# thiviyanT/ARK

Hardware: AMD Instinct MI355X
Metric: training graphs/sec (higher is better)
Workload: dtype f16 fwd / bf16 bwd MFMA operands (BASELINE configs[1] says bf16: bf16 forward operands miss the 1e-4 ELBO bar, fp16 has the same width and MFMA rate), f32 accumulate+state; 1 GPU; autoreg_syn-paths SAIL train step (fwd+ELBO+bwd+Adam; batches resident in HBM); batch_per_gpu=1024, global_batch=1024, d_model=512, d_latent=10, n_layers=3, seq_len=11, vocab=55, hipgraph=True, launch=hipGraph replay, settle_steps=300, parallelism=dp1

## Files before the change

### ark_amd/csrc/embed.hip

```cpp
#include "common.h"
#include "../../include/ark_amd.h"

namespace ark {

__device__ __forceinline__ void put16x4(void* base, long idx4, f32x4 v, int prec) {
  if (prec == PREC_F16) {
    typedef _Float16 h4 __attribute__((ext_vector_type(4)));
    auto c = [](float x) { return (_Float16)fminf(fmaxf(x, -65504.0f), 65504.0f); };
    reinterpret_cast<h4*>(base)[idx4] = h4{c(v[0]), c(v[1]), c(v[2]), c(v[3])};
  } else {
    typedef __bf16 b4 __attribute__((ext_vector_type(4)));
    reinterpret_cast<b4*>(base)[idx4] = b4{(__bf16)v[0], (__bf16)v[1], (__bf16)v[2], (__bf16)v[3]};
  }
}

__device__ __forceinline__ void enc_pool_fwd_body(int b, const int64_t* __restrict__ triples, const float* __restrict__ E,
                                                           const float* __restrict__ R, float* __restrict__ g,
                                                           float* __restrict__ inv_cnt, int T, int D, long pad_rid,
                                                           void* g16a, int prec_a, void* g16b, int prec_b) {
  const int64_t* tr = triples + (long)b * T * 3;
  int cnt = 0;
  for (int t = 0; t < T; ++t) cnt += (pad_rid < 0 || tr[t * 3 + 1] != pad_rid) ? 1 : 0;
  const float w = 1.0f / (float)(pad_rid < 0 ? T : (cnt > 0 ? cnt : 1));
  if (threadIdx.x == 0 && inv_cnt) inv_cnt[b] = w;
// ... 191 lines not shown
      id[k] = 0; srow[k] = 0; sc[k] = 0.f;
      ok[k] = (i + k < i1) && scatter_item(p, i + k, id[k], srow[k], sc[k]) && col_ok;
    }
#pragma unroll
    for (int k = 0; k < U; ++k) v[k] = ok[k] ? p.src[srow[k] * p.ld_src + p.col_off + c0 + lane] : 0.f;
#pragma unroll
    for (int k = 0; k < U; ++k)
      if (ok[k]) atomicAdd(&tab[id[k] * 64 + lane], sc[k] * v[k]);
  }
  __syncthreads();
  if (col_ok)
    for (int r = wave; r < p.n_rows; r += 4) {
      const float v = tab[r * 64 + lane];
      if (v != 0.f) atomicAdd(&p.dst[(long)r * p.D + c0 + lane], v);
    }
}

__global__ __launch_bounds__(256) void scatter_global_kernel(ScatterArgs p) {
  const int lane = threadIdx.x & 63;
  const int wave_global = blockIdx.x * 4 + (threadIdx.x >> 6);
  const int n_waves = gridDim.x * 4;
  for (int i = wave_global; i < p.n_items; i += n_waves) {
    long id, srow; float sc;
    if (!scatter_item(p, i, id, srow, sc)) continue;
    const float* s = p.src + srow * p.ld_src + p.col_off;
    float* d = p.dst + id * p.D;
    for (int c = lane; c < p.D; c += 64) {
      const float v = sc * s[c];
      if (v != 0.f) atomicAdd(&d[c], v);
    }
  }
}

__global__ __launch_bounds__(256) void enc_scatter_fused_kernel(const int64_t* __restrict__ triples, const float* __restrict__ dg,
                                                                const float* __restrict__ inv_cnt, float* __restrict__ dE,
                                                                float* __restrict__ dR, int B, int T, int D, int n_ent, int n_rel,
                                                                long pad_eid, long pad_rid, int n_chunks) {
  ARK_CHAIN_PRIO();
  extern __shared__ __attribute__((aligned(16))) char smem[];
  float* te = reinterpret_cast<float*>(smem);
  float* tr = te + (size_t)n_ent * 64;
  const int slice = blockIdx.x / n_chunks, chunk = blockIdx.x % n_chunks;
  const int c0 = slice * 64;
  const int lane = threadIdx.x & 63, wave = threadIdx.x >> 6;
  for (int i = threadIdx.x; i < (n_ent + n_rel) * 64; i += 256) te[i] = 0.f;
  __syncthreads();
  const int n_items = B * T;
  const int per = (n_items + n_chunks - 1) / n_chunks;
  const int i0 = chunk * per, i1 = min(n_items, i0 + per);
  const bool col_ok = (c0 + lane) < D;
  constexpr int U = 4;
  for (int i = i0 + wave * U; i < i1; i += 4 * U) {
    long h[U], r[U], t[U]; float sc[U], vh[U], vr[U], vt[U]; bool ok[U];
#pragma unroll
    for (int k = 0; k < U; ++k) {
      const int it = min(i + k, i1 - 1);
      const int64_t* p3 = triples + (long)it * 3;
      h[k] = p3[0]; r[k] = p3[1]; t[k] = p3[2];
      ok[k] = (i + k < i1) && col_ok && !(pad_rid >= 0 && r[k] == pad_rid);
      sc[k] = inv_cnt[it / T];
    }
#pragma unroll
    for (int k = 0; k < U; ++k) {
      const int it = min(i + k, i1 - 1);
      const float* src = dg + (long)(it / T) * 3 * D + c0 + lane;
      vh[k] = ok[k] ? src[0] : 0.f; vr[k] = ok[k] ? src[D] : 0.f; vt[k] = ok[k] ? src[2 * D] : 0.f;
    }
#pragma unroll
    for (int k = 0; k < U; ++k)
      if (ok[k]) {
        if (h[k] != pad_eid) atomicAdd(&te[h[k] * 64 + lane], sc[k] * vh[k]);
        if (r[k] != pad_rid) atomicAdd(&tr[r[k] * 64 + lane], sc[k] * vr[k]);
        if (t[k] != pad_eid) atomicAdd(&te[t[k] * 64 + lane], sc[k] * vt[k]);
      }
  }
  __syncthreads();
  if (col_ok) {
    for (int row = wave; row < n_ent; row += 4) {
      const float v = te[row * 64 + lane];
      if (v != 0.f) atomicAdd(&dE[(long)row * D + c0 + lane], v);
    }
    for (int row = wave; row < n_rel; row += 4) {
      const float v = tr[row * 64 + lane];
      if (v != 0.f) atomicAdd(&dR[(long)row * D + c0 + lane], v);
    }
  }
}

#ifndef ARK_SCATTER_CHUNK
#define ARK_SCATTER_CHUNK 48
#endif
constexpr int g_scatter_chunk_items = ARK_SCATTER_CHUNK;

static int launch_scatter(const ScatterArgs& p, hipStream_t st) {
  if (p.n_items <= 0) return 0;
  if ((long)p.n_rows * 64 * 4 <= 48 * 1024) {
    const int slices = (p.D + 63) / 64;
    int n_chunks = (p.n_items + g_scatter_chunk_items - 1) / g_scatter_chunk_items;
    if (n_chunks > 2048 / slices) n_chunks = 2048 / slices;
    if (n_chunks < 1) n_chunks = 1;
    hipLaunchKernelGGL(scatter_lds_kernel, dim3(slices * n_chunks), dim3(256), (size_t)p.n_rows * 64 * 4, st, p, n_chunks);
  } else {
    int grid = (p.n_items + 3) / 4; if (grid > 2048) grid = 2048;
    hipLaunchKernelGGL(scatter_global_kernel, dim3(grid), dim3(256), 0, st, p);
  }
  ARK_LAUNCH_CHECK();
  return 0;
}

}

extern "C" int ark_enc_pool_fwd(const int64_t* triples, const float* E, const float* R, float* g, float* inv_cnt,
                                int B, int T, int D, int64_t pad_rid, void* stream) {
  using namespace ark;
  if (!triples || !E || !R || !g || B <= 0 || T <= 0 || D <= 0) return ARK_ERR_ARG;
  if (D % 4 != 0) return ARK_ERR_SHAPE;
  hipLaunchKernelGGL(enc_pool_fwd_kernel, dim3(B), dim3(256), 0, (hipStream_t)stream, triples, E, R, g, inv_cnt, T, D,
// ... 28 lines not shown
  if (x16a && (g16b == nullptr) != (x16b == nullptr)) return ARK_ERR_ARG;
  PoolGatherArgs p{triples, E, R, g, inv_cnt, g16a, g16b, seq, w_tok, x16a, x16b, hyper_tick, tok_tm, (long)pad_rid, (long)ld_seq,
                   B, T, D, D_dec, L, prec_a, prec_b, 0};
  const long total = x16a ? (long)B * L * (D_dec / 4) : (long)B * L;
  long gb = (total + 255) / 256; if (gb > 4096) gb = 4096; if (gb < 1) gb = 1;
  size_t lds = 0;
  if (T >= 32 && (long)B * ((3 * (D / 4) + 63) / 64) <= 2048) {
    p.col_blocks = (3 * (D / 4) + 63) / 64;
    lds = (size_t)((T * 3 * 8 + 15) / 16) * 16 + 4 * 64 * 16;
    if (lds > 60 * 1024) { p.col_blocks = 0; lds = 0; }
  }
  const long npool = p.col_blocks > 0 ? (long)B * p.col_blocks : B;
  hipLaunchKernelGGL(pool_gather_fwd_kernel, dim3((unsigned)(npool + gb)), dim3(256), lds, (hipStream_t)stream, p);
  ARK_LAUNCH_CHECK();
  return 0;
}

extern "C" int ark_tok_time_major(const int64_t* seq, int64_t ld_seq, int* tok_tm, int B, int L, float* hyper_tick, void* stream) {
  if (!seq || !tok_tm || B <= 0 || L <= 0) return ARK_ERR_ARG;
  const long rows = (long)B * L;
  long gb = (rows + 255) / 256; if (gb > 1024) gb = 1024;
  hipLaunchKernelGGL(ark::tok_time_major_kernel, dim3((unsigned)gb), dim3(256), 0, (hipStream_t)stream, seq, (long)ld_seq, tok_tm, B, L,
                     hyper_tick);
  ARK_LAUNCH_CHECK();
  return 0;
}

extern "C" int ark_enc_pool_bwd(const int64_t* triples, const float* dg, const float* inv_cnt, float* dE, float* dR,
                                int B, int T, int D, int n_ent, int n_rel, int64_t pad_eid, int64_t pad_rid,
                                void* stream) {
  using namespace ark;
  if (!triples || !dg || !inv_cnt || !dE || !dR || B <= 0 || T <= 0 || D <= 0) return ARK_ERR_ARG;
  hipStream_t st = (hipStream_t)stream;
  if ((long)(n_ent + n_rel) * 64 * 4 <= 48 * 1024) {
    const int slices = (D + 63) / 64;
    int n_chunks = (B * T + g_scatter_chunk_items - 1) / g_scatter_chunk_items;
    if (n_chunks > 2048 / slices) n_chunks = 2048 / slices;
    if (n_chunks < 1) n_chunks = 1;
    hipLaunchKernelGGL(enc_scatter_fused_kernel, dim3(slices * n_chunks), dim3(256), (size_t)(n_ent + n_rel) * 64 * 4, st,
                       triples, dg, inv_cnt, dE, dR, B, T, D, n_ent, n_rel, (long)pad_eid, (long)pad_rid, n_chunks);
    ARK_LAUNCH_CHECK();
    return 0;
  }
  for (int part = 0; part < 3; ++part) {
    ScatterArgs p{};
    p.dst = (part == 1) ? dR : dE; p.src = dg; p.ld_src = 3L * D; p.col_off = part * D;
    p.ids = triples; p.id_stride_outer = 3L * T; p.id_stride_inner = 3; p.inner = T; p.id_off = part;
    p.mask_ids = pad_rid >= 0 ? triples : nullptr; p.mask_off = 1; p.mask_val = (long)pad_rid;
    p.scale = inv_cnt; p.src_div = T; p.time_major = 0; p.n_outer = B;
    p.skip_id = (part == 1) ? (long)pad_rid : (long)pad_eid;
    p.n_items = B * T; p.D = D; p.n_rows = (part == 1) ? n_rel : n_ent;
    int rc = launch_scatter(p, st);
    if (rc) return rc;
  }
  return 0;
}

extern "C" int ark_tok_gather(const int64_t* seq, int64_t ld_seq, const float* w_tok, const float* w_pos, float* x,
                              int B, int L, int D, float* hyper_tick, void* stream) {
  using namespace ark;
  if (!seq || !w_tok || !x || B <= 0 || L <= 0 || D <= 0) return ARK_ERR_ARG;
  if (D % 4 != 0) return ARK_ERR_SHAPE;
  long total = (long)B * L * (D / 4);
  int grid = (int)((total + 255) / 256); if (grid > 4096) grid = 4096;
  hipLaunchKernelGGL(tok_gather_kernel, dim3(grid), dim3(256), 0, (hipStream_t)stream, seq, (long)ld_seq, w_tok, w_pos,
                     x, B, L, D, hyper_tick);
  ARK_LAUNCH_CHECK();
  return 0;
}

extern "C" int ark_tok_scatter(const int64_t* seq, int64_t ld_seq, const float* dx, float* d_w_tok, int B, int L, int D,
                               int vocab, void* stream) {
  using namespace ark;
// ... 9 lines not shown
```

### ark_amd/csrc/loss.hip

```cpp
#include "common.h"
#include "../../include/ark_amd.h"

namespace ark {

__device__ __forceinline__ float block_sum_1024(float v, float* red) {
  v = wave_sum(v);
  const int lane = threadIdx.x & 63, wave = threadIdx.x >> 6;
  if (lane == 0) red[wave] = v;
  __syncthreads();
  float t = 0.f;
  if (wave == 0) {
    t = (lane < (int)(blockDim.x >> 6)) ? red[lane] : 0.f;
    t = wave_sum(t);
  }
  __syncthreads();
  return t;
}

__global__ __launch_bounds__(1024) void latent_fwd_kernel(const float* __restrict__ head, const float* __restrict__ eps,
                                                          float* __restrict__ mu, float* __restrict__ logv,
                                                          float* __restrict__ z, float* __restrict__ kl_out, int B, int Z,
                                                          int clamp) {
  __shared__ float red[16];
  float acc = 0.f;
// ... 199 lines not shown
  if constexpr (!BATCHED) {
    const int row0 = blockIdx.x * RW;
    constexpr int KC = 3;
    for (int cb = 0; cb < H; cb += 256 * KC) {
      float acc4[KC][RW];
  #pragma unroll
      for (int k = 0; k < KC; ++k)
  #pragma unroll
        for (int r = 0; r < RW; ++r) acc4[k][r] = 0.f;
  #pragma unroll
      for (int j = 0; j < 2 * ZT; ++j)
        if (j < 2 * Z) {
          float dj[RW];
  #pragma unroll
          for (int r = 0; r < RW; ++r) dj[r] = sh[r][j];
  #pragma unroll
          for (int k = 0; k < KC; ++k) {
            const int c = cb + 256 * k + threadIdx.x;
            const float wv = (c < H) ? Whead[(long)j * H + c] : 0.f;
  #pragma unroll
            for (int r = 0; r < RW; ++r) acc4[k][r] += dj[r] * wv;
          }
        }
  #pragma unroll
      for (int k = 0; k < KC; ++k) {
        const int c = cb + 256 * k + threadIdx.x;
        if (c >= H) continue;
        float cs = 0.f;
  #pragma unroll
        for (int r = 0; r < RW; ++r) {
          if (row0 + r >= B) break;
          const long o = (long)(row0 + r) * H + c;
          const float v = acc4[k][r] * dgelu_erf(pre[o]);
          dA[o] = v;
          cs += v;
          if (prec16 == 2) reinterpret_cast<_Float16*>(dA16)[o] = (_Float16)fminf(fmaxf(v, -65504.f), 65504.f);
          else reinterpret_cast<__bf16*>(dA16)[o] = (__bf16)v;
        }
        if (dA_colsum) atomicAdd(&dA_colsum[c], cs);
      }
    }
  } else {
    const int row0 = blockIdx.x * RW;
    constexpr int KC = 3, JC = 16;
    static_assert((2 * ZT) % JC == 0, "batches of head rows");
    for (int cb = 0; cb < H; cb += 256 * KC) {
      float acc4[KC][RW], pv[KC][RW];
  #pragma unroll
      for (int k = 0; k < KC; ++k)
  #pragma unroll
        for (int r = 0; r < RW; ++r) {
          acc4[k][r] = 0.f;
          const int c = cb + 256 * k + threadIdx.x;
          pv[k][r] = (c < H && row0 + r < B) ? pre[(long)(row0 + r) * H + c] : 0.f;
        }
  #pragma unroll 1
      for (int j0 = 0; j0 < 2 * Z; j0 += JC) {
        float wv[JC][KC];
  #pragma unroll
        for (int jj = 0; jj < JC; ++jj)
  #pragma unroll
          for (int k = 0; k < KC; ++k) {
            const int c = cb + 256 * k + threadIdx.x;
            wv[jj][k] = (j0 + jj < 2 * Z && c < H) ? Whead[(long)(j0 + jj) * H + c] : 0.f;
          }
  #pragma unroll
        for (int jj = 0; jj < JC; ++jj) {
          float dj[RW];
  #pragma unroll
          for (int r = 0; r < RW; ++r) dj[r] = (j0 + jj < 2 * Z) ? sh[r][j0 + jj] : 0.f;
  #pragma unroll
          for (int k = 0; k < KC; ++k)
  #pragma unroll
            for (int r = 0; r < RW; ++r) acc4[k][r] += dj[r] * wv[jj][k];
        }
      }
  #pragma unroll
      for (int k = 0; k < KC; ++k) {
        const int c = cb + 256 * k + threadIdx.x;
        if (c >= H) continue;
        float cs = 0.f;
  #pragma unroll
        for (int r = 0; r < RW; ++r) {
          if (row0 + r >= B) break;
          const long o = (long)(row0 + r) * H + c;
          const float v = acc4[k][r] * dgelu_erf(pv[k][r]);
          dA[o] = v;
          cs += v;
          if (prec16 == 2) reinterpret_cast<_Float16*>(dA16)[o] = (_Float16)fminf(fmaxf(v, -65504.f), 65504.f);
          else reinterpret_cast<__bf16*>(dA16)[o] = (__bf16)v;
        }
        if (dA_colsum) atomicAdd(&dA_colsum[c], cs);
      }
    }
  }
}

template <int ZT, int DU>
__global__ __launch_bounds__(256) void latent_dz_head_kernel(float* __restrict__ dh0, const float* __restrict__ h0,
                                                             const float* __restrict__ Wz, const float* __restrict__ head,
                                                             const float* __restrict__ eps, const float* __restrict__ hyper,
                                                             const float* __restrict__ ext_dhead, float* __restrict__ dhead,
                                                             int B, int Z, int D) {
  ARK_CHAIN_PRIO();
  extern __shared__ __attribute__((aligned(16))) char smem_dz[];
  float* zs = reinterpret_cast<float*>(smem_dz);
  const int wave = threadIdx.x >> 6, lane = threadIdx.x & 63;
  const int DS = D + 1;
  const int b = (int)blockIdx.x * 4 + wave;
  const bool valid = b < B;
  const int bb = valid ? b : B - 1;
  float hv[DU], gv[DU];
#pragma unroll
  for (int u = 0; u < DU; ++u) {
    const int d = lane + 64 * u;
    hv[u] = d < D ? h0[(long)bb * D + d] : 0.f;
    gv[u] = d < D ? dh0[(long)bb * D + d] : 0.f;
  }
  {
    const int N4 = (D * Z) >> 2;
// ... 27 lines not shown
    const int d = lane + 64 * u;
    if (d < D) {
      const float g = gv[u] * (1.0f - hv[u] * hv[u]);
      if (valid) dh0[(long)bb * D + d] = g;
#pragma unroll
      for (int j = 0; j < ZT; ++j)
        if (j < Z) acc[j] += g * zs[j * DS + d];
    }
  }
  float mydz = 0.f;
#pragma unroll
  for (int j = 0; j < ZT; ++j)
    if (j < Z) {
      const float a = wave_sum(acc[j]);
      if (lane == j) mydz = a;
    }
  if (lane < Z && valid) {
    const float ks = hyper[ARK_HP_BETA] * hyper[ARK_HP_KL_NORM];
    const float m = head[(long)b * 2 * Z + lane];
    const float raw = head[(long)b * 2 * Z + Z + lane];
    const float lv = fminf(fmaxf(raw, -10.0f), 10.0f);
    float dmu = mydz + ks * m;
    float dlv = mydz * (eps ? eps[(long)b * Z + lane] : 0.f) * 0.5f * expf(0.5f * lv) + ks * 0.5f * (expf(lv) - 1.0f);
    if (raw < -10.0f || raw > 10.0f) dlv = 0.f;
    if (ext_dhead) {
      dmu += ext_dhead[(long)b * 2 * Z + lane];
      dlv += ext_dhead[(long)b * 2 * Z + Z + lane];
    }
    dhead[(long)b * 2 * Z + lane] = dmu;
    dhead[(long)b * 2 * Z + Z + lane] = dlv;
  }
}

__global__ __launch_bounds__(256) void latent_dA_kernel(const float* __restrict__ dhead, const float* __restrict__ Whead,
                                                        const float* __restrict__ pre, float* __restrict__ dA, void* dA16, int prec16,
                                                        float* __restrict__ dA_colsum, int B, int Z2, int H) {
  ARK_CHAIN_PRIO();
  constexpr int RW = 8;
  __shared__ float sh[RW][256];
  const int row0 = blockIdx.x * RW;
  const int Z2p = (Z2 + 31) & ~31;
  for (int i = threadIdx.x; i < RW * Z2p; i += 256) {
    const int r = i / Z2p, j = i - r * Z2p;
    sh[r][j] = (row0 + r < B && j < Z2) ? dhead[(long)(row0 + r) * Z2 + j] : 0.f;
  }
  __syncthreads();
  const int c = blockIdx.y * 256 + threadIdx.x;
  if (c >= H) return;
  float acc[RW], pv[RW];
#pragma unroll
  for (int r = 0; r < RW; ++r) {
    acc[r] = 0.f;
    pv[r] = row0 + r < B ? pre[(long)(row0 + r) * H + c] : 0.f;
  }
  for (int j0 = 0; j0 < Z2; j0 += 32) {
    float wv[32];
#pragma unroll
    for (int u = 0; u < 32; ++u) wv[u] = Whead[(long)min(j0 + u, Z2 - 1) * H + c];
#pragma unroll
    for (int u = 0; u < 32; ++u) {
#pragma unroll
      for (int r = 0; r < RW; ++r) acc[r] += sh[r][j0 + u] * wv[u];
    }
  }
  float cs = 0.f;
#pragma unroll
  for (int r = 0; r < RW; ++r) {
    if (row0 + r >= B) break;
    const long o = (long)(row0 + r) * H + c;
    const float v = acc[r] * dgelu_erf(pv[r]);
    dA[o] = v;
    cs += v;
    if (prec16 == 2) reinterpret_cast<_Float16*>(dA16)[o] = (_Float16)fminf(fmaxf(v, -65504.f), 65504.f);
    else reinterpret_cast<__bf16*>(dA16)[o] = (__bf16)v;
  }
  if (dA_colsum) atomicAdd(&dA_colsum[c], cs);
}

template <int ZT>
__global__ __launch_bounds__(256) void zproj_bwd_dw_kernel(const float* __restrict__ dzp, const float* __restrict__ z,
                                                           float* __restrict__ dWz, float* __restrict__ dbz, int B, int Z,
                                                           int D, int b_chunk) {
  extern __shared__ __attribute__((aligned(16))) char smem_z[];
  float* zs = reinterpret_cast<float*>(smem_z);
  float* red = zs + (size_t)b_chunk * ZT;
  const int lane = threadIdx.x & 63, rg = threadIdx.x >> 6;
  const int d = blockIdx.x * 64 + lane;
  const int b0 = blockIdx.y * b_chunk, nb = min(B, b0 + b_chunk) - b0;
  for (int i = threadIdx.x; i < b_chunk * ZT; i += 256) {
    const int bb = i / ZT, j = i % ZT;
    zs[i] = (bb < nb && j < Z) ? z[(long)(b0 + bb) * Z + j] : 0.f;
  }
  __syncthreads();
  float acc[ZT];
#pragma unroll
  for (int j = 0; j < ZT; ++j) acc[j] = 0.f;
  float sb = 0.f;
  if (d < D)
    for (int bb = rg; bb < nb; bb += 4) {
      const float g = dzp[(long)(b0 + bb) * D + d];
      sb += g;
#pragma unroll
      for (int j = 0; j < ZT; ++j) acc[j] += g * zs[bb * ZT + j];
    }
#pragma unroll
  for (int j = 0; j <= ZT; ++j) {
    const float v = (j < ZT) ? acc[j < ZT ? j : 0] : sb;
    red[rg * 64 + lane] = v;
    __syncthreads();
    if (rg == 0 && d < D) {
      const float t = red[lane] + red[64 + lane] + red[128 + lane] + red[192 + lane];
      if (j < ZT) { if (j < Z) atomicAdd(&dWz[(long)d * Z + j], t); }
      else atomicAdd(&dbz[d], t);
    }
    __syncthreads();
  }
}

struct LatentReduceArgs {
  const float* dzp; const float* z; float* dWz; float* dbz;
  const float* dhead; const void* act16; int prec16; float* dWh; float* dbh;
  int B, Z, D, H, b_chunk;
};

template <int ZT>
__global__ __launch_bounds__(256) void latent_reduce_bwd_kernel(LatentReduceArgs p) {
  extern __shared__ __attribute__((aligned(16))) char smem_lr[];
  float* zs = reinterpret_cast<float*>(smem_lr);
  float* red = zs + (size_t)p.b_chunk * ZT;
  const int job = blockIdx.z;
  const int jbase = job == 0 ? 0 : (job - 1) * ZT;
  const int NTOT = job == 0 ? p.Z : 2 * p.Z;
  const int NW = job == 0 ? p.D : p.H, NS = min(NTOT - jbase, ZT);
  if ((int)blockIdx.x * 64 >= NW) return;
  const float* skinny = (job == 0 ? p.z : p.dhead) + jbase;
  const int lane = threadIdx.x & 63, rg = threadIdx.x >> 6;
  const int c = blockIdx.x * 64 + lane;
  const int b0 = blockIdx.y * p.b_chunk, nb = min(p.B, b0 + p.b_chunk) - b0;
  for (int i = threadIdx.x; i < p.b_chunk * ZT; i += 256) {
    const int bb = i / ZT, j = i % ZT;
    zs[i] = (bb < nb && j < NS) ? skinny[(long)(b0 + bb) * NTOT + j] : 0.f;
  }
  __syncthreads();
  float acc[ZT];
#pragma unroll
  for (int j = 0; j < ZT; ++j) acc[j] = 0.f;
  float sb = 0.f;
  if (c < NW)
    for (int bb = rg; bb < nb; bb += 4) {
      float g;
      if (job == 0) g = p.dzp[(long)(b0 + bb) * p.D + c];
      else if (p.prec16 == PREC_F16) g = (float)reinterpret_cast<const _Float16*>(p.act16)[(long)(b0 + bb) * p.H + c];
      else g = (float)reinterpret_cast<const __bf16*>(p.act16)[(long)(b0 + bb) * p.H + c];
      sb += g;
#pragma unroll
      for (int j = 0; j < ZT; ++j) acc[j] += g * zs[bb * ZT + j];
    }
#pragma unroll
  for (int j = 0; j <= ZT; ++j) {
    if (j < ZT && j >= NS) continue;
    if (j == ZT && job != 0) continue;
    const float v = (j < ZT) ? acc[j < ZT ? j : 0] : sb;
    red[rg * 64 + lane] = v;
    __syncthreads();
    if (rg == 0 && c < NW) {
      const float t = red[lane] + red[64 + lane] + red[128 + lane] + red[192 + lane];
      if (j == ZT) atomicAdd(&p.dbz[c], t);
      else if (job == 0) atomicAdd(&p.dWz[(long)c * p.Z + j], t);
      else atomicAdd(&p.dWh[(long)(jbase + j) * p.H + c], t);
    }
    __syncthreads();
  }
  if (job >= 1 && blockIdx.x == 0 && (int)threadIdx.x < NS) {
    float t = 0.f;
    for (int bb = 0; bb < nb; ++bb) t += zs[bb * ZT + threadIdx.x];
    atomicAdd(&p.dbh[jbase + threadIdx.x], t);
  }
}

__global__ __launch_bounds__(256) void ce_kernel(float* logits, long ld, const int64_t* __restrict__ seq,
                                                 long ld_seq, const float* __restrict__ hyper, float* __restrict__ row_loss,
                                                 float* dlogits, __bf16* d16bf, _Float16* d16h, long ld16, int B, int L, int V) {
  const int row = blockIdx.x * 4 + (threadIdx.x >> 6), lane = threadIdx.x & 63;
  if (row >= B * L) return;
  const int t = row / B, b = row % B;
  const long tgt = seq[(long)b * ld_seq + t + 1];
  const float* x = logits + (long)row * ld;
  float mx = -INFINITY;
  for (int c = lane; c < V; c += 64) mx = fmaxf(mx, x[c]);
  mx = wave_max(mx);
  float se = 0.f;
  for (int c = lane; c < V; c += 64) se += expf(x[c] - mx);
  se = wave_sum(se);
  const float lse = mx + logf(se);
  const bool live = (tgt != ARK_TOK_PAD);
  if (lane == 0) row_loss[row] = live ? (lse - x[tgt]) : 0.f;
  if (dlogits || d16bf || d16h) {
    const float s = live ? hyper[ARK_HP_CE_INV_COUNT] : 0.f;
    float* d = dlogits ? dlogits + (long)row * ld : nullptr;
    const long nc = (d16bf || d16h) ? ((ld16 > ld || !d) ? ld16 : ld) : ld;
    for (int c = lane; c < nc; c += 64) {
      float g = 0.f;
      if (c < V) g = (expf(x[c] - lse) - ((long)c == tgt ? 1.0f : 0.f)) * s;
      if (d && c < ld) d[c] = g;
      if (c < ld16) {
        if (d16bf) d16bf[(long)row * ld16 + c] = (__bf16)g;
// ... 212 lines not shown
  ARK_LAUNCH_CHECK();
  return 0;
}

extern "C" int ark_zproj_bwd_dw(const float* dzp, const float* z, float* d_w_z, float* d_b_z, int B, int Z, int D,
                                int accumulate, void* stream) {
  using namespace ark;
  if (!dzp || !z || !d_w_z || !d_b_z || B <= 0 || Z <= 0 || D <= 0) return ARK_ERR_ARG;
  if (Z > 128) return ARK_ERR_SHAPE;
  hipStream_t st = (hipStream_t)stream;
  if (!accumulate) {
    hipError_t e = hipMemsetAsync(d_w_z, 0, sizeof(float) * (size_t)D * Z, st);
    if (e != hipSuccess) return (int)e;
    e = hipMemsetAsync(d_b_z, 0, sizeof(float) * (size_t)D, st);
    if (e != hipSuccess) return (int)e;
  }
  const int b_chunk = 32;
  dim3 grid((D + 63) / 64, (B + b_chunk - 1) / b_chunk);
#define ARK_ZDW(ZT) hipLaunchKernelGGL(zproj_bwd_dw_kernel<ZT>, grid, dim3(256), (size_t)(b_chunk * ZT + 256) * sizeof(float), st, dzp, z, d_w_z, d_b_z, B, Z, D, b_chunk)
  if (Z <= 16) ARK_ZDW(16);
  else if (Z <= 32) ARK_ZDW(32);
  else if (Z <= 64) ARK_ZDW(64);
  else ARK_ZDW(128);
#undef ARK_ZDW
  ARK_LAUNCH_CHECK();
  return 0;
}

extern "C" int ark_latent_chain_bwd(float* dh0, const float* h0, const float* w_z, const float* head, const float* eps,
                                    const float* hyper, const float* ext_dhead, const float* w_head, const float* pre,
                                    float* dhead, float* dA, void* dA16, int prec16, float* dA_colsum, int B, int Z, int D, int H,
                                    void* stream) {
  using namespace ark;
  if (!dh0 || !h0 || !w_z || !head || !hyper || !w_head || !pre || !dhead || !dA || !dA16 || B <= 0 || Z <= 0 || D <= 0 || H <= 0)
    return ARK_ERR_ARG;
  if (Z > 128) return ARK_ERR_SHAPE;
  if (prec16 != 1 && prec16 != 2) return ARK_ERR_ARG;
  hipStream_t st = (hipStream_t)stream;
  const size_t lds = Z > 64 ? (size_t)(D + 256) * sizeof(float)
                            : (size_t)Z * (D + 1) * sizeof(float);
  if (lds > 150 * 1024) return ARK_ERR_SHAPE;
#ifndef ARK_NO_LATENT_DZ
  if (Z <= 32 && D % 4 == 0 && D <= 1024 && B >= 64 && H >= 768) {
    const size_t l2 = (size_t)Z * (D + 1) * sizeof(float);
#define ARK_DZ(ZT, DU)                                                                                                       \
    {                                                                                                                        \
      static bool once = ((void)hipFuncSetAttribute(reinterpret_cast<const void*>(latent_dz_head_kernel<ZT, DU>),            \
                                                    hipFuncAttributeMaxDynamicSharedMemorySize, 150 * 1024), true);         \
      (void)once;                                                                                                            \
      hipLaunchKernelGGL((latent_dz_head_kernel<ZT, DU>), dim3((B + 3) / 4), dim3(256), l2, st, dh0, h0, w_z, head, eps, hyper, \
                         ext_dhead, dhead, B, Z, D);                                                                         \
    }
    if (l2 <= 150 * 1024) {
      if (Z <= 16 && D <= 512) ARK_DZ(16, 8)
      else if (Z <= 16) ARK_DZ(16, 16)
      else if (D <= 512) ARK_DZ(32, 8)
      else ARK_DZ(32, 16)
#undef ARK_DZ
      ARK_LAUNCH_CHECK();
      hipLaunchKernelGGL(latent_dA_kernel, dim3((B + 7) / 8, (H + 255) / 256), dim3(256), 0, st, dhead, w_head, pre, dA, dA16, prec16,
                         dA_colsum, B, 2 * Z, H);
      ARK_LAUNCH_CHECK();
      return 0;
    }
  }
#endif
  const bool split = Z <= 64 && (B + 3) / 4 < 128 && H >= 768;
  const int Hc = split ? 0 : H;
#define ARK_LC(ZT)                                                                                                          \
  {                                                                                                                         \
    static bool once = ((void)hipFuncSetAttribute(reinterpret_cast<const void*>(latent_chain_bwd_kernel<ZT, 4, (ZT > 32)>),            \
                                                  hipFuncAttributeMaxDynamicSharedMemorySize, 150 * 1024), true);           \
    (void)once;                                                                                                             \
    hipLaunchKernelGGL((latent_chain_bwd_kernel<ZT, 4, (ZT > 32)>), dim3((B + 3) / 4), dim3(256), lds, st, dh0, h0, w_z, head, eps,     \
                       hyper, ext_dhead, w_head, pre, dhead, dA, dA16, prec16, dA_colsum, B, Z, D, Hc);                                 \
  }
  if (Z <= 16) ARK_LC(16)
  else if (Z <= 32) ARK_LC(32)
  else if (Z <= 64) ARK_LC(64)
  else {
    if (D % 2 != 0) return ARK_ERR_SHAPE;
    static bool once = ((void)hipFuncSetAttribute(reinterpret_cast<const void*>(latent_chain_bwd_kernel<128, 1, true>),
                                                  hipFuncAttributeMaxDynamicSharedMemorySize, 150 * 1024), true);
    (void)once;
    hipLaunchKernelGGL((latent_chain_bwd_kernel<128, 1, true>), dim3(B), dim3(256), lds, st, dh0, h0, w_z, head, eps, hyper,
                       ext_dhead, w_head, pre, dhead, dA, dA16, prec16, dA_colsum, B, Z, D, H);
  }
#undef ARK_LC
  ARK_LAUNCH_CHECK();
  if (split) {
    hipLaunchKernelGGL(latent_dA_kernel, dim3((B + 7) / 8, (H + 255) / 256), dim3(256), 0, st, dhead, w_head, pre, dA, dA16, prec16,
                       dA_colsum, B, 2 * Z, H);
    ARK_LAUNCH_CHECK();
  }
  return 0;
}

extern "C" int ark_latent_reduce_bwd(const float* dzp, const float* z, float* d_w_z, float* d_b_z, const float* dhead,
                                     const void* act16, int prec16, float* d_w_head, float* d_b_head, int B, int Z, int D, int H,
                                     void* stream) {
  using namespace ark;
  if (!dzp || !z || !d_w_z || !d_b_z || !dhead || !act16 || !d_w_head || !d_b_head || B <= 0 || Z <= 0 || D <= 0 || H <= 0)
    return ARK_ERR_ARG;
  if (prec16 != PREC_F16 && prec16 != PREC_BF16) return ARK_ERR_ARG;
  if (Z > 128) return ARK_ERR_SHAPE;
  LatentReduceArgs p{dzp, z, d_w_z, d_b_z, dhead, act16, prec16, d_w_head, d_b_head, B, Z, D, H, 32};
  const int wide = D > H ? D : H;
  const int zt = 2 * Z <= 32 ? 32 : 2 * Z <= 64 ? 64 : 128;
  dim3 grid((wide + 63) / 64, (B + p.b_chunk - 1) / p.b_chunk, 1 + (2 * Z + zt - 1) / zt);
  hipStream_t st = (hipStream_t)stream;
#define ARK_LR(ZT) hipLaunchKernelGGL(latent_reduce_bwd_kernel<ZT>, grid, dim3(256), (size_t)(p.b_chunk * ZT + 256) * sizeof(float), st, p)
  if (2 * Z <= 32) ARK_LR(32);
  else if (2 * Z <= 64) ARK_LR(64);
  else ARK_LR(128);
#undef ARK_LR
  ARK_LAUNCH_CHECK();
  return 0;
}

extern "C" int ark_count_targets(const int64_t* seq, int64_t ld_seq, int B, int L, float* hyper, void* stream) {
  using namespace ark;
  if (!seq || !hyper || B <= 0 || L <= 0) return ARK_ERR_ARG;
  hipLaunchKernelGGL(count_targets_kernel, dim3(1), dim3(1024), 0, (hipStream_t)stream, seq, (long)ld_seq, B, L, hyper);
  ARK_LAUNCH_CHECK();
  return 0;
}

extern "C" int ark_ce_fwd_bwd(float* logits, int64_t ld, const int64_t* seq, int64_t ld_seq, const float* hyper,
                              float* row_loss, float* dlogits, void* dlogits16, int prec16, int64_t ld16, int B, int L, int V,
                              void* stream) {
  using namespace ark;
  if (!logits || !seq || !hyper || !row_loss || B <= 0 || L <= 0 || V <= 0 || ld < V) return ARK_ERR_ARG;
  if (dlogits16 && (ld16 < V || (prec16 != 1 && prec16 != 2))) return ARK_ERR_ARG;
  __bf16* dbf = prec16 == 1 ? (__bf16*)dlogits16 : nullptr;
  _Float16* dh = prec16 == 2 ? (_Float16*)dlogits16 : nullptr;
  const size_t ld_bytes = (size_t)ld * sizeof(float);
  if (V >= 4096 && ld_bytes <= 144 * 1024 && ld % 4 == 0) {
    const int nr = (int)((ld / 4 + 1023) / 1024);
    int grid = 256 * 1;
    if (grid > B * L) grid = B * L;
#define ARK_CE_LDS(NRV)                                                                                                   \
    {                                                                                                                     \
// ... 44 lines not shown
```

### ark_amd/engine.py

```python
import math
from collections import OrderedDict

import torch

from . import _lib as L

HP = dict(LR=0, BETA=1, KL_NORM=2, CE_INV_COUNT=3, CE_COUNT=4, ADAM_STEP=5, ADAM_BC1=6, ADAM_BC2=7, ADAM_B1=8,
          ADAM_B2=9, ADAM_EPS=10, GRAD_SCALE=11, DROP_STEP=12, NOISE_STEP=13, COUNT=16)

PREC = {"f32": (L.PREC_F32, L.PREC_F32), "fp32": (L.PREC_F32, L.PREC_F32), "float32": (L.PREC_F32, L.PREC_F32),
        "bf16": (L.PREC_BF16, L.PREC_BF16), "bfloat16": (L.PREC_BF16, L.PREC_BF16),
        "f16": (L.PREC_F16, L.PREC_F16), "mixed": (L.PREC_F16, L.PREC_BF16)}


def _rup(x, m):
    return (x + m - 1) // m * m


CAPTURE_MODE = "thread_local"

_calls = [0]


def _ranks_on_this_device(world_size):
# ... 990 lines not shown
            return True
        if self._finalize is not None:
            self._finalize()
            self._finalize = None
        self._zero(self.G)
        dX0 = self._backward_decoder_v1(w, B, Lq, seq, use_drop)
        _call("ark_tok_scatter", L.ptr(seq), L.i64(ld_seq), L.ptr(dX0), L.ptr(g["dec.tok_emb.weight"]), L.i32(B), L.i32(Lq),
              L.i32(D), L.i32(V), st)
        if self.mt == "ARK":
            gp = g["dec.pos_emb.weight"]
            self._colsum(dX0, D, gp, B, D, n_batch=Lq, bs_in=B * D, bs_out=D)
            self._join_side()
            return False
        return True

    def backward_encoder(self, ext_dhead=None):
        self.prec = self.prec_bwd
        w, B, T, Lq = self.ws, self._B, self._T, self._Lrun
        D, n, V, Z = self.D, self.n, self.V, self.Z
        st = L.cur_stream()
        KM, MM = L.LAY_KMAJ, L.LAY_MMAJ
        p, g = self.p, self.g
        nv = self._n_valid
        H = 3 * D
        h0rm = w["h0"] if w["v2"] else w["Y"][0]
        fused = w["v2"] and Z <= 128
        if fused:
            pb = self.prec_bwd
            a16b = lambda i: (w["act16b"][i] if w["act16b"][i] is not None else w["act16a"][i])
            g16b = w["g16b"] if w["g16b"] is not None else w["g16a"]
            ext = ext_dhead.contiguous() if ext_dhead is not None else None
            _call("ark_latent_chain_bwd", L.ptr(w["dH0"]), L.ptr(h0rm), L.ptr(p["dec.z_proj.weight"]), L.ptr(w["head"]),
                  L.ptr(self._eps), L.ptr(self.hyper), L.ptr(ext), L.ptr(p["enc.mu.weight"]), L.ptr(w["pre"][n - 1]),
                  L.ptr(w["dhead"]), L.ptr(w["dA"]), L.ptr(w["dpre16"][n - 1]), L.i32(pb),
                  L.ptr(g[f"enc.mlp.{2 * (n - 1)}.bias"]), L.i32(nv), L.i32(Z), L.i32(D), L.i32(H), st)
            if self._ce_dw_pending is not None and not self.ce_dw_last:
                self._ce_dw_pending()
                self._ce_dw_pending = None
            if self._fork_pending is not None:
                self._fork_pending()
            main = torch.cuda.current_stream()
            side = self._side_stream() if self.overlap_wgrad else main
            if self._side_heavy():
                side = main
            side.wait_stream(main)
            with torch.cuda.stream(side):
                ss = L.cur_stream()
                _call("ark_latent_reduce_bwd", L.ptr(w["dH0"]), L.ptr(w["z"]), L.ptr(g["dec.z_proj.weight"]),
                      L.ptr(g["dec.z_proj.bias"]), L.ptr(w["dhead"]), L.ptr(a16b(n - 1)), L.i32(pb), L.ptr(g["enc.mu.weight"]),
                      L.ptr(g["enc.mu.bias"]), L.i32(nv), L.i32(Z), L.i32(D), L.i32(H), ss)
            self._side_used = self._side_used or (side is not main)
        else:
            if self._ce_dw_pending is not None:
                self._ce_dw_pending()
                self._ce_dw_pending = None
            if self._fork_pending is not None:
                self._fork_pending()
            _call("ark_zproj_bwd", L.ptr(w["dH0"]), L.ptr(h0rm), L.ptr(w["z"]), L.ptr(p["dec.z_proj.weight"]),
                  L.ptr(w["dz"]), L.ptr(g["dec.z_proj.weight"]), L.ptr(g["dec.z_proj.bias"]), L.i32(B), L.i32(Z), L.i32(D), L.i32(1), st)
            _call("ark_latent_bwd", L.ptr(w["dz"]), L.ptr(w["head"]), L.ptr(self._eps), L.ptr(self.hyper), L.ptr(w["dhead"]),
                  L.i32(B), L.i32(Z), st)
            if ext_dhead is not None:
                w["dhead"].add_(ext_dhead)
            self._colsum(w["dhead"], 2 * Z, g["enc.mu.bias"], B, 2 * Z)
        if w["v2"]:
            pb = self.prec_bwd
            a16b = lambda i: (w["act16b"][i] if w["act16b"][i] is not None else w["act16a"][i])
# ... 808 lines not shown
```

### include/ark_amd.h

```cpp
#ifndef ARK_AMD_H
#define ARK_AMD_H
#include <stdint.h>
#ifdef __cplusplus
extern "C" {
#endif

#define ARK_PREC_F32 0
#define ARK_PREC_BF16 1
#define ARK_PREC_F16 2
#define ARK_LAY_KMAJ 0
#define ARK_LAY_MMAJ 1

#define ARK_EPI_NONE 0
#define ARK_EPI_BIAS 1
#define ARK_EPI_BIAS_GELU 2
#define ARK_EPI_MUL_DGELU 3
#define ARK_EPI_MUL_AUX 4
#define ARK_EPI_BIAS_RELU 5
#define ARK_EPI_MUL_RELU 6
#define ARK_EPI_ADD 7

int ark_version(void);

int ark_gemm(int prec, int a_lay, int b_lay, int epi, const float* A, int64_t lda, const float* B, int64_t ldb,
// ... 197 lines not shown
               const float* hyper, void* stream);
int ark_uncast16(int prec, const void* x16, float* out, int64_t n, void* stream);
int ark_to_tiled(const float* x, float* out, int rows, int ld, void* stream);
int ark_from_tiled(const float* x, float* out, int rows, int ld, void* stream);

int ark_enc_pool_fwd(const int64_t* triples, const float* E, const float* R, float* g, float* inv_cnt, int B, int T,
                     int D, int64_t pad_rid , void* stream);
int ark_enc_pool_fwd16(const int64_t* triples, const float* E, const float* R, float* g, float* inv_cnt, void* g16a,
                       int prec_a, void* g16b, int prec_b, int B, int T, int D, int64_t pad_rid, void* stream);
int ark_enc_pool_bwd(const int64_t* triples, const float* dg, const float* inv_cnt, float* dE, float* dR, int B,
                     int T, int D, int n_ent, int n_rel, int64_t pad_eid, int64_t pad_rid, void* stream);
int ark_tok_gather(const int64_t* seq, int64_t ld_seq, const float* w_tok, const float* w_pos ,
                   float* x, int B, int L, int D, float* hyper_tick , void* stream);
int ark_pool_gather_fwd16(const int64_t* triples, const float* E, const float* R, float* g, float* inv_cnt, void* g16a,
                          int prec_a, void* g16b, int prec_b, int B, int T, int D, int64_t pad_rid, const int64_t* seq,
                          int64_t ld_seq, const float* w_tok, void* x16a, void* x16b, int L, int D_dec, int* tok_tm,
                          float* hyper_tick, void* stream);
int ark_tok_time_major(const int64_t* seq, int64_t ld_seq, int* tok_tm, int B, int L, float* hyper_tick, void* stream);
int ark_tok_scatter(const int64_t* seq, int64_t ld_seq, const float* dx, float* d_w_tok, int B, int L, int D,
                    int vocab, void* stream);

int ark_latent_fwd(const float* head , const float* eps ,
                   float* mu, float* logv, float* z, float* kl_out, int B, int Z, void* stream);
int ark_latent_bwd(const float* dz, const float* head, const float* eps, const float* hyper, float* dhead, int B,
                   int Z, void* stream);
int ark_zproj_fwd(const float* z, const float* w_z, const float* b_z, float* h0, int64_t copy_stride, int n_copies,
                  int B, int Z, int D, void* stream);
int ark_zproj_bwd(float* dh0, const float* h0, const float* z, const float* w_z, float* dz, float* d_w_z,
                  float* d_b_z, int B, int Z, int D, int accumulate, void* stream);
int ark_zproj_bwd_dw(const float* dzp, const float* z, float* d_w_z, float* d_b_z, int B, int Z, int D, int accumulate,
                     void* stream);
int ark_latent_chain_bwd(float* dh0, const float* h0, const float* w_z, const float* head, const float* eps,
                         const float* hyper, const float* ext_dhead , const float* w_head ,
                         const float* pre , float* dhead, float* dA, void* dA16, int prec16,
                         float* dA_colsum ,
                         int B, int Z, int D, int H, void* stream);
int ark_latent_reduce_bwd(const float* dzp, const float* z, float* d_w_z, float* d_b_z, const float* dhead, const void* act16,
                          int prec16, float* d_w_head, float* d_b_head, int B, int Z, int D, int H, void* stream);
int ark_count_targets(const int64_t* seq, int64_t ld_seq, int B, int L, float* hyper, void* stream);
int ark_ce_fwd_bwd(float* logits, int64_t ld, const int64_t* seq, int64_t ld_seq, const float* hyper,
                   float* row_loss, float* dlogits, void* dlogits16, int prec16, int64_t ld16, int B, int L, int V,
                   void* stream);
int ark_vocab_ce_fwd(int prec, const void* Y16, const void* W16, const float* bias, const int64_t* seq, int64_t ld_seq,
                     const float* hyper, float* row_loss, float* lse, float* dY_t , int B, int L, int V, int D,
                     void* stream);
int ark_vocab_ce_fwd_splits(int R, int V, int D, int cu_budget);
int ark_vocab_ce_fwd_ws(int prec, const void* Y16, const void* W16, const float* bias, const int64_t* seq, int64_t ld_seq,
                        const float* hyper, float* row_loss, float* lse, float* dY_t, float* ws, int64_t ws_floats, int B,
                        int L, int V, int D, int cu_budget, void* stream);
int ark_vocab_ce_dw(int prec, const void* Y16, const void* W16, const float* bias, const int64_t* seq, int64_t ld_seq,
                    const float* hyper, const float* lse, float* dW, float* db, int B, int L, int V, int D, void* stream);
int ark_loss_finalize(const float* row_loss, int n_rows, const float* kl, const float* hyper, float* out4,
                      void* stream);
int ark_loss_finalize_rows(const float* row_loss, int n_rows, const float* kl_rows, int n_kl, float kl_scale,
                           const float* hyper, float* out4, void* stream);
int ark_argmax_rows(const float* x, int64_t ld, int64_t* out, int rows, int V, void* stream);

int ark_layernorm_fwd(const float* x, const float* res, const float* gamma, const float* beta, float* s_out, float* y,
                      float* stats, int rows, int D, float eps, void* stream);
int ark_layernorm_fwd_drop(const float* x, const float* res, const float* gamma, const float* beta, float* s_out, float* y,
                           float* stats, int rows, int D, float eps, float drop_p, uint64_t seed, const float* hyper, void* stream);
int ark_layernorm_bwd(const float* dy, const float* s, const float* stats, const float* gamma, float* ds, float* dgamma,
                      float* dbeta, int rows, int D, void* stream);
int ark_dropout_apply(float* x, int64_t n, float p, uint64_t seed, const float* hyper, void* stream);
int ark_attn_fwd(const float* qkv, float* out, float* probs, const unsigned char* kmask ,
                 int B, int L, int D, int n_heads, int causal, float drop_p, uint64_t seed, const float* hyper, void* stream);
int ark_attn_bwd(const float* qkv, const float* out, const float* probs, const float* dout, float* dscore, float* dqkv,
// ... 47 lines not shown
```

Baseline: 961,800 graphs/s.

## Retune encoder scatter, latent dA, and latent reduce kernels; drop unused f32 dA store

The encoder pooling backward scatter now uses 8-column slices with 32 items in flight per thread group and int indices with pad sentinels, which gives many more blocks and smaller LDS tiles. The latent dA kernel drops its shared-memory staging, becomes templated on rows per block with a vectorized path, and gets a launcher that picks 8 or 16 rows. The latent reduce kernel flattens its jobs onto grid.x, sizes the batch chunk to fill about 256 blocks, and unrolls its batch loop by 4. The fp32 dA write is made optional and the engine passes null, since only the 16-bit copy is consumed. Together these aim to raise parallelism and cut memory traffic in small backward kernels, at the cost of more global atomics and redundant reads of dhead.

New measurement: 945,100 graphs/s. -1.7%, worse.

```diff
diff --git a/ark_amd/csrc/embed.hip b/ark_amd/csrc/embed.hip
--- a/ark_amd/csrc/embed.hip
+++ b/ark_amd/csrc/embed.hip
@@ -247,57 +247,60 @@
   }
 }
 
+constexpr int kEncScatterCols = 8;
+constexpr int kEncScatterChunks = 2;
 __global__ __launch_bounds__(256) void enc_scatter_fused_kernel(const int64_t* __restrict__ triples, const float* __restrict__ dg,
                                                                 const float* __restrict__ inv_cnt, float* __restrict__ dE,
                                                                 float* __restrict__ dR, int B, int T, int D, int n_ent, int n_rel,
                                                                 long pad_eid, long pad_rid, int n_chunks) {
   ARK_CHAIN_PRIO();
+  constexpr int C = kEncScatterCols, IW = 64 / C, U = 8;
   extern __shared__ __attribute__((aligned(16))) char smem[];
   float* te = reinterpret_cast<float*>(smem);
-  float* tr = te + (size_t)n_ent * 64;
+  float* tr = te + (size_t)n_ent * C;
   const int slice = blockIdx.x / n_chunks, chunk = blockIdx.x % n_chunks;
-  const int c0 = slice * 64;
-  const int lane = threadIdx.x & 63, wave = threadIdx.x >> 6;
-  for (int i = threadIdx.x; i < (n_ent + n_rel) * 64; i += 256) te[i] = 0.f;
+  const int c0 = slice * C;
+  const int col = threadIdx.x % C, sub = threadIdx.x / C;
+  for (int i = threadIdx.x; i < (n_ent + n_rel) * C; i += 256) te[i] = 0.f;
   __syncthreads();
   const int n_items = B * T;
   const int per = (n_items + n_chunks - 1) / n_chunks;
   const int i0 = chunk * per, i1 = min(n_items, i0 + per);
-  const bool col_ok = (c0 + lane) < D;
-  constexpr int U = 4;
-  for (int i = i0 + wave * U; i < i1; i += 4 * U) {
-    long h[U], r[U], t[U]; float sc[U], vh[U], vr[U], vt[U]; bool ok[U];
+  const bool col_ok = (c0 + col) < D;
+  for (int i = i0 + sub; i < i1; i += 4 * IW * U) {
+    int h[U], r[U], t[U]; float sc[U], vh[U], vr[U], vt[U]; bool ok[U];
 #pragma unroll
     for (int k = 0; k < U; ++k) {
-      const int it = min(i + k, i1 - 1);
+      const int it = min(i + 4 * IW * k, i1 - 1);
       const int64_t* p3 = triples + (long)it * 3;
-      h[k] = p3[0]; r[k] = p3[1]; t[k] = p3[2];
-      ok[k] = (i + k < i1) && col_ok && !(pad_rid >= 0 && r[k] == pad_rid);
+      const long hl = p3[0], rl = p3[1], tl = p3[2];
+      ok[k] = (i + 4 * IW * k < i1) && col_ok && !(pad_rid >= 0 && rl == pad_rid);
+      h[k] = hl == pad_eid ? -1 : (int)hl; r[k] = rl == pad_rid ? -1 : (int)rl; t[k] = tl == pad_eid ? -1 : (int)tl;
       sc[k] = inv_cnt[it / T];
     }
 #pragma unroll
     for (int k = 0; k < U; ++k) {
-      const int it = min(i + k, i1 - 1);
-      const float* src = dg + (long)(it / T) * 3 * D + c0 + lane;
+      const int it = min(i + 4 * IW * k, i1 - 1);
+      const float* src = dg + (long)(it / T) * 3 * D + c0 + col;
       vh[k] = ok[k] ? src[0] : 0.f; vr[k] = ok[k] ? src[D] : 0.f; vt[k] = ok[k] ? src[2 * D] : 0.f;
     }
 #pragma unroll
     for (int k = 0; k < U; ++k)
       if (ok[k]) {
-        if (h[k] != pad_eid) atomicAdd(&te[h[k] * 64 + lane], sc[k] * vh[k]);
-        if (r[k] != pad_rid) atomicAdd(&tr[r[k] * 64 + lane], sc[k] * vr[k]);
-        if (t[k] != pad_eid) atomicAdd(&te[t[k] * 64 + lane], sc[k] * vt[k]);
+        if (h[k] >= 0) atomicAdd(&te[h[k] * C + col], sc[k] * vh[k]);
+        if (r[k] >= 0) atomicAdd(&tr[r[k] * C + col], sc[k] * vr[k]);
+        if (t[k] >= 0) atomicAdd(&te[t[k] * C + col], sc[k] * vt[k]);
       }
   }
   __syncthreads();
   if (col_ok) {
-    for (int row = wave; row < n_ent; row += 4) {
-      const float v = te[row * 64 + lane];
-      if (v != 0.f) atomicAdd(&dE[(long)row * D + c0 + lane], v);
-    }
-    for (int row = wave; row < n_rel; row += 4) {
-      const float v = tr[row * 64 + lane];
-      if (v != 0.f) atomicAdd(&dR[(long)row * D + c0 + lane], v);
+    for (int row = sub; row < n_ent; row += 4 * IW) {
+      const float v = te[row * C + col];
+      if (v != 0.f) atomicAdd(&dE[(long)row * D + c0 + col], v);
+    }
+    for (int row = sub; row < n_rel; row += 4 * IW) {
+      const float v = tr[row * C + col];
+      if (v != 0.f) atomicAdd(&dR[(long)row * D + c0 + col], v);
     }
   }
 }
@@ -392,13 +395,12 @@
   using namespace ark;
   if (!triples || !dg || !inv_cnt || !dE || !dR || B <= 0 || T <= 0 || D <= 0) return ARK_ERR_ARG;
   hipStream_t st = (hipStream_t)stream;
-  if ((long)(n_ent + n_rel) * 64 * 4 <= 48 * 1024) {
-    const int slices = (D + 63) / 64;
-    int n_chunks = (B * T + g_scatter_chunk_items - 1) / g_scatter_chunk_items;
-    if (n_chunks > 2048 / slices) n_chunks = 2048 / slices;
-    if (n_chunks < 1) n_chunks = 1;
-    hipLaunchKernelGGL(enc_scatter_fused_kernel, dim3(slices * n_chunks), dim3(256), (size_t)(n_ent + n_rel) * 64 * 4, st,
-                       triples, dg, inv_cnt, dE, dR, B, T, D, n_ent, n_rel, (long)pad_eid, (long)pad_rid, n_chunks);
+  if (n_ent + n_rel <= 192) {
+    const int slices = (D + kEncScatterCols - 1) / kEncScatterCols;
+    const int n_chunks = (long)B * T > 256 ? kEncScatterChunks : 1;
+    hipLaunchKernelGGL(enc_scatter_fused_kernel, dim3(slices * n_chunks), dim3(256),
+                       (size_t)(n_ent + n_rel) * kEncScatterCols * sizeof(float), st, triples, dg, inv_cnt, dE, dR, B, T, D, n_ent,
+                       n_rel, (long)pad_eid, (long)pad_rid, n_chunks);
     ARK_LAUNCH_CHECK();
     return 0;
   }
diff --git a/ark_amd/csrc/loss.hip b/ark_amd/csrc/loss.hip
--- a/ark_amd/csrc/loss.hip
+++ b/ark_amd/csrc/loss.hip
@@ -255,7 +255,7 @@
           if (row0 + r >= B) break;
           const long o = (long)(row0 + r) * H + c;
           const float v = acc4[k][r] * dgelu_erf(pre[o]);
-          dA[o] = v;
+          if (dA) dA[o] = v;
           cs += v;
           if (prec16 == 2) reinterpret_cast<_Float16*>(dA16)[o] = (_Float16)fminf(fmaxf(v, -65504.f), 65504.f);
           else reinterpret_cast<__bf16*>(dA16)[o] = (__bf16)v;
@@ -308,7 +308,7 @@
           if (row0 + r >= B) break;
           const long o = (long)(row0 + r) * H + c;
           const float v = acc4[k][r] * dgelu_erf(pv[k][r]);
-          dA[o] = v;
+          if (dA) dA[o] = v;
           cs += v;
           if (prec16 == 2) reinterpret_cast<_Float16*>(dA16)[o] = (_Float16)fminf(fmaxf(v, -65504.f), 65504.f);
           else reinterpret_cast<__bf16*>(dA16)[o] = (__bf16)v;
@@ -402,49 +402,76 @@
   }
 }
 
-__global__ __launch_bounds__(256) void latent_dA_kernel(const float* __restrict__ dhead, const float* __restrict__ Whead,
-                                                        const float* __restrict__ pre, float* __restrict__ dA, void* dA16, int prec16,
-                                                        float* __restrict__ dA_colsum, int B, int Z2, int H) {
+template <int RW, bool V4>
+__global__ __launch_bounds__(256, 5) void latent_dA_kernel(const float* __restrict__ dhead, const float* __restrict__ Whead,
+                                                           const float* __restrict__ pre, float* __restrict__ dA, void* dA16,
+                                                           int prec16, float* __restrict__ dA_colsum, int B, int Z2, int H) {
   ARK_CHAIN_PRIO();
-  constexpr int RW = 8;
-  __shared__ float sh[RW][256];
+  constexpr int JB = 32;
   const int row0 = blockIdx.x * RW;
-  const int Z2p = (Z2 + 31) & ~31;
-  for (int i = threadIdx.x; i < RW * Z2p; i += 256) {
-    const int r = i / Z2p, j = i - r * Z2p;
-    sh[r][j] = (row0 + r < B && j < Z2) ? dhead[(long)(row0 + r) * Z2 + j] : 0.f;
-  }
-  __syncthreads();
   const int c = blockIdx.y * 256 + threadIdx.x;
   if (c >= H) return;
-  float acc[RW], pv[RW];
-#pragma unroll
-  for (int r = 0; r < RW; ++r) {
-    acc[r] = 0.f;
-    pv[r] = row0 + r < B ? pre[(long)(row0 + r) * H + c] : 0.f;
-  }
-  for (int j0 = 0; j0 < Z2; j0 += 32) {
-    float wv[32];
-#pragma unroll
-    for (int u = 0; u < 32; ++u) wv[u] = Whead[(long)min(j0 + u, Z2 - 1) * H + c];
-#pragma unroll
-    for (int u = 0; u < 32; ++u) {
-#pragma unroll
-      for (int r = 0; r < RW; ++r) acc[r] += sh[r][j0 + u] * wv[u];
+  float acc[RW];
+#pragma unroll
+  for (int r = 0; r < RW; ++r) acc[r] = 0.f;
+#pragma unroll 1
+  for (int j0 = 0; j0 < Z2; j0 += JB) {
+    float wv[JB];
+#pragma unroll
+    for (int u = 0; u < JB; ++u) wv[u] = Whead[(long)min(j0 + u, Z2 - 1) * H + c];
+#pragma unroll
+    for (int r = 0; r < RW; ++r) {
+      const float* d = dhead + (long)min(row0 + r, B - 1) * Z2;
+      if constexpr (V4) {
+#pragma unroll
+        for (int u = 0; u < JB; u += 4) {
+          const bool in = j0 + u < Z2;
+          const float* q = d + min(j0 + u, Z2 - 4);
+          const float s0 = q[0], s1 = q[1], s2 = q[2], s3 = q[3];
+          acc[r] += (in ? s0 : 0.f) * wv[u];
+          acc[r] += (in ? s1 : 0.f) * wv[u + 1];
+          acc[r] += (in ? s2 : 0.f) * wv[u + 2];
+          acc[r] += (in ? s3 : 0.f) * wv[u + 3];
+        }
+      } else {
+#pragma unroll
+        for (int u = 0; u < JB; ++u) {
+          const float s = j0 + u < Z2 ? d[min(j0 + u, Z2 - 1)] : 0.f;
+          acc[r] += s * wv[u];
+        }
+      }
     }
   }
   float cs = 0.f;
-#pragma unroll
-  for (int r = 0; r < RW; ++r) {
-    if (row0 + r >= B) break;
-    const long o = (long)(row0 + r) * H + c;
-    const float v = acc[r] * dgelu_erf(pv[r]);
-    dA[o] = v;
-    cs += v;
-    if (prec16 == 2) reinterpret_cast<_Float16*>(dA16)[o] = (_Float16)fminf(fmaxf(v, -65504.f), 65504.f);
-    else reinterpret_cast<__bf16*>(dA16)[o] = (__bf16)v;
+  constexpr int PB = 4;
+#pragma unroll
+  for (int r0 = 0; r0 < RW; r0 += PB) {
+    float pv[PB];
+#pragma unroll
+    for (int r = 0; r < PB; ++r) pv[r] = row0 + r0 + r < B ? pre[(long)(row0 + r0 + r) * H + c] : 0.f;
+#pragma unroll
+    for (int r = 0; r < PB; ++r) {
+      if (row0 + r0 + r >= B) break;
+      const long o = (long)(row0 + r0 + r) * H + c;
+      const float v = acc[r0 + r] * dgelu_erf(pv[r]);
+      if (dA) dA[o] = v;
+      cs += v;
+      if (prec16 == 2) reinterpret_cast<_Float16*>(dA16)[o] = (_Float16)fminf(fmaxf(v, -65504.f), 65504.f);
+      else reinterpret_cast<__bf16*>(dA16)[o] = (__bf16)v;
+    }
   }
   if (dA_colsum) atomicAdd(&dA_colsum[c], cs);
+}
+
+static void launch_latent_dA(const float* dhead, const float* w_head, const float* pre, float* dA, void* dA16, int prec16,
+                             float* dA_colsum, int B, int Z2, int H, hipStream_t st) {
+  const int cb = (H + 255) / 256;
+  const bool r8 = (long)((B + 7) / 8) * cb <= 512;
+  const dim3 grid(r8 ? (B + 7) / 8 : (B + 15) / 16, cb);
+#define ARK_DA(RWV, V4V) hipLaunchKernelGGL((latent_dA_kernel<RWV, V4V>), grid, dim3(256), 0, st, dhead, w_head, pre, dA, dA16, prec16, dA_colsum, B, Z2, H)
+  if (Z2 % 4 == 0) { if (r8) ARK_DA(8, true); else ARK_DA(16, true); }
+  else { if (r8) ARK_DA(8, false); else ARK_DA(16, false); }
+#undef ARK_DA
 }
 
 template <int ZT>
@@ -498,14 +525,15 @@
   extern __shared__ __attribute__((aligned(16))) char smem_lr[];
   float* zs = reinterpret_cast<float*>(smem_lr);
   float* red = zs + (size_t)p.b_chunk * ZT;
-  const int job = blockIdx.z;
+  const int nd = (p.D + 63) / 64, nh = (p.H + 63) / 64;
+  const int job = (int)blockIdx.x < nd ? 0 : 1 + ((int)blockIdx.x - nd) / nh;
+  const int cblk = job == 0 ? (int)blockIdx.x : ((int)blockIdx.x - nd) % nh;
   const int jbase = job == 0 ? 0 : (job - 1) * ZT;
   const int NTOT = job == 0 ? p.Z : 2 * p.Z;
   const int NW = job == 0 ? p.D : p.H, NS = min(NTOT - jbase, ZT);
-  if ((int)blockIdx.x * 64 >= NW) return;
   const float* skinny = (job == 0 ? p.z : p.dhead) + jbase;
   const int lane = threadIdx.x & 63, rg = threadIdx.x >> 6;
-  const int c = blockIdx.x * 64 + lane;
+  const int c = cblk * 64 + lane;
   const int b0 = blockIdx.y * p.b_chunk, nb = min(p.B, b0 + p.b_chunk) - b0;
   for (int i = threadIdx.x; i < p.b_chunk * ZT; i += 256) {
     const int bb = i / ZT, j = i % ZT;
@@ -517,14 +545,24 @@
   for (int j = 0; j < ZT; ++j) acc[j] = 0.f;
   float sb = 0.f;
   if (c < NW)
-    for (int bb = rg; bb < nb; bb += 4) {
-      float g;
-      if (job == 0) g = p.dzp[(long)(b0 + bb) * p.D + c];
-      else if (p.prec16 == PREC_F16) g = (float)reinterpret_cast<const _Float16*>(p.act16)[(long)(b0 + bb) * p.H + c];
-      else g = (float)reinterpret_cast<const __bf16*>(p.act16)[(long)(b0 + bb) * p.H + c];
-      sb += g;
-#pragma unroll
-      for (int j = 0; j < ZT; ++j) acc[j] += g * zs[bb * ZT + j];
+    for (int b4 = rg; b4 < nb; b4 += 16) {
+      float g[4];
+#pragma unroll
+      for (int u = 0; u < 4; ++u) {
+        const int bb = b4 + 4 * u;
+        const long row = b0 + min(bb, nb - 1);
+        if (job == 0) g[u] = p.dzp[row * p.D + c];
+        else if (p.prec16 == PREC_F16) g[u] = (float)reinterpret_cast<const _Float16*>(p.act16)[row * p.H + c];
+        else g[u] = (float)reinterpret_cast<const __bf16*>(p.act16)[row * p.H + c];
+        if (bb >= nb) g[u] = 0.f;
+      }
+#pragma unroll
+      for (int u = 0; u < 4; ++u) {
+        const int bb = min(b4 + 4 * u, nb - 1);
+        sb += g[u];
+#pragma unroll
+        for (int j = 0; j < ZT; ++j) acc[j] += g[u] * zs[bb * ZT + j];
+      }
     }
 #pragma unroll
   for (int j = 0; j <= ZT; ++j) {
@@ -541,7 +579,7 @@
     }
     __syncthreads();
   }
-  if (job >= 1 && blockIdx.x == 0 && (int)threadIdx.x < NS) {
+  if (job >= 1 && cblk == 0 && (int)threadIdx.x < NS) {
     float t = 0.f;
     for (int bb = 0; bb < nb; ++bb) t += zs[bb * ZT + threadIdx.x];
     atomicAdd(&p.dbh[jbase + threadIdx.x], t);
@@ -820,7 +858,7 @@
                                     float* dhead, float* dA, void* dA16, int prec16, float* dA_colsum, int B, int Z, int D, int H,
                                     void* stream) {
   using namespace ark;
-  if (!dh0 || !h0 || !w_z || !head || !hyper || !w_head || !pre || !dhead || !dA || !dA16 || B <= 0 || Z <= 0 || D <= 0 || H <= 0)
+  if (!dh0 || !h0 || !w_z || !head || !hyper || !w_head || !pre || !dhead || !dA16 || B <= 0 || Z <= 0 || D <= 0 || H <= 0)
     return ARK_ERR_ARG;
   if (Z > 128) return ARK_ERR_SHAPE;
   if (prec16 != 1 && prec16 != 2) return ARK_ERR_ARG;
@@ -846,8 +884,7 @@
       else ARK_DZ(32, 16)
 #undef ARK_DZ
       ARK_LAUNCH_CHECK();
-      hipLaunchKernelGGL(latent_dA_kernel, dim3((B + 7) / 8, (H + 255) / 256), dim3(256), 0, st, dhead, w_head, pre, dA, dA16, prec16,
-                         dA_colsum, B, 2 * Z, H);
+      launch_latent_dA(dhead, w_head, pre, dA, dA16, prec16, dA_colsum, B, 2 * Z, H, st);
       ARK_LAUNCH_CHECK();
       return 0;
     }
@@ -877,8 +914,7 @@
 #undef ARK_LC
   ARK_LAUNCH_CHECK();
   if (split) {
-    hipLaunchKernelGGL(latent_dA_kernel, dim3((B + 7) / 8, (H + 255) / 256), dim3(256), 0, st, dhead, w_head, pre, dA, dA16, prec16,
-                       dA_colsum, B, 2 * Z, H);
+    launch_latent_dA(dhead, w_head, pre, dA, dA16, prec16, dA_colsum, B, 2 * Z, H, st);
     ARK_LAUNCH_CHECK();
   }
   return 0;
@@ -893,9 +929,16 @@
   if (prec16 != PREC_F16 && prec16 != PREC_BF16) return ARK_ERR_ARG;
   if (Z > 128) return ARK_ERR_SHAPE;
   LatentReduceArgs p{dzp, z, d_w_z, d_b_z, dhead, act16, prec16, d_w_head, d_b_head, B, Z, D, H, 32};
-  const int wide = D > H ? D : H;
   const int zt = 2 * Z <= 32 ? 32 : 2 * Z <= 64 ? 64 : 128;
-  dim3 grid((wide + 63) / 64, (B + p.b_chunk - 1) / p.b_chunk, 1 + (2 * Z + zt - 1) / zt);
+  const int per_chunk = (D + 63) / 64 + ((H + 63) / 64) * ((2 * Z + zt - 1) / zt);
+  {
+    const int n_chunks = 256 / per_chunk > 1 ? 256 / per_chunk : 1;
+    int bc = ((B + n_chunks - 1) / n_chunks + 3) & ~3;
+    if (bc < 32) bc = 32;
+    if (bc > 8192 / zt) bc = 8192 / zt;
+    p.b_chunk = bc;
+  }
+  dim3 grid(per_chunk, (B + p.b_chunk - 1) / p.b_chunk);
   hipStream_t st = (hipStream_t)stream;
 #define ARK_LR(ZT) hipLaunchKernelGGL(latent_reduce_bwd_kernel<ZT>, grid, dim3(256), (size_t)(p.b_chunk * ZT + 256) * sizeof(float), st, p)
   if (2 * Z <= 32) ARK_LR(32);
diff --git a/ark_amd/engine.py b/ark_amd/engine.py
--- a/ark_amd/engine.py
+++ b/ark_amd/engine.py
@@ -1046,7 +1046,7 @@
             ext = ext_dhead.contiguous() if ext_dhead is not None else None
             _call("ark_latent_chain_bwd", L.ptr(w["dH0"]), L.ptr(h0rm), L.ptr(p["dec.z_proj.weight"]), L.ptr(w["head"]),
                   L.ptr(self._eps), L.ptr(self.hyper), L.ptr(ext), L.ptr(p["enc.mu.weight"]), L.ptr(w["pre"][n - 1]),
-                  L.ptr(w["dhead"]), L.ptr(w["dA"]), L.ptr(w["dpre16"][n - 1]), L.i32(pb),
+                  L.ptr(w["dhead"]), L.ptr(None), L.ptr(w["dpre16"][n - 1]), L.i32(pb),
                   L.ptr(g[f"enc.mlp.{2 * (n - 1)}.bias"]), L.i32(nv), L.i32(Z), L.i32(D), L.i32(H), st)
             if self._ce_dw_pending is not None and not self.ce_dw_last:
                 self._ce_dw_pending()
diff --git a/include/ark_amd.h b/include/ark_amd.h
--- a/include/ark_amd.h
+++ b/include/ark_amd.h
@@ -253,7 +253,7 @@
                      void* stream);
 int ark_latent_chain_bwd(float* dh0, const float* h0, const float* w_z, const float* head, const float* eps,
                          const float* hyper, const float* ext_dhead , const float* w_head ,
-                         const float* pre , float* dhead, float* dA, void* dA16, int prec16,
+                         const float* pre , float* dhead, float* dA , void* dA16, int prec16,
                          float* dA_colsum ,
                          int B, int Z, int D, int H, void* stream);
 int ark_latent_reduce_bwd(const float* dzp, const float* z, float* d_w_z, float* d_b_z, const float* dhead, const void* act16,
```
